# HuiGuanLab/Lite-MKD

Measured on AMD Instinct MI355X. Metric: episodes/sec (5-way 5-shot, 8x224^2 frames), higher is better.
Workload: dtype f32

## Files before the change

### include/lmkd.h

```cpp
#ifndef LMKD_H
#define LMKD_H
#ifdef __cplusplus
extern "C" {
#endif

int lmkd_abi_version(void);
const char* lmkd_last_error(void);
int lmkd_device_check(int device);
int lmkd_set_activation_dtype(int mode);
int lmkd_get_activation_dtype(void);

int lmkd_gemm_f32(char layA, char layB, int M, int N, int K, float alpha, const float* A, long lda, long sA,
                  const float* B, long ldb, long sB, float beta, float* C, long ldc, long sC, const float* bias,
                  int relu, int batch, void* stream);
int lmkd_gemm_set_mode(int mode);
int lmkd_gemm_set_tile(int t);
long lmkd_gemm_ticket_words(void);
int lmkd_gemm_f32_splitk(char layA, char layB, int M, int N, int K, float alpha, const float* A, long lda, long sA,
                         const float* B, long ldb, long sB, float beta, float* C, long ldc, long sC, const float* bias,
                         int relu, int batch, void* workspace, long ws_bytes, unsigned* tickets, void* stream);

long lmkd_conv2d_packed_weight_elems(int Cout, int Cin, int Cs, int KH, int KW, int mode);
int lmkd_conv2d_pack_weights(const float* w_oihw, float* wp, int Cout, int Cin, int Cs, int KH, int KW, int mode ,
                             void* stream);
int lmkd_conv2d_fwd_row_tiles(int N, int H, int W, int Cout, int KH, int KW, int stride, int pad);
int lmkd_conv2d_fwd_row_tiles_cs(int N, int H, int W, int Cs, int Cout, int KH, int KW, int stride, int pad);
int lmkd_set_elementwise_wg_per_cu(int n);
int lmkd_conv_set_compute_dtype(int mode);
typedef struct lmkd_amax_desc {
  const void* x_words;
  const void* dy_words;
  void* out_words;
  const void* ref_words;
  int flags;
} lmkd_amax_desc;
#define LMKD_AMAX_FENCED 1
int lmkd_h2_fence_eval(const void* const* words, void* const* refs, int n, int* flags, void* stream);
long lmkd_conv_h2_fallbacks(void);
int lmkd_amax(const float* x, long n, void* word, void* stream);
long lmkd_amax_words(void);
long lmkd_conv2d_plane_elems(int ncols, int Kp);
long lmkd_conv_h2_launches(void);
int lmkd_conv2d_repack_multi(const float* const* ws, void* const* wfs, const int* dims, int n, void* stream);
int lmkd_conv2d_split_weights(const float* wp, void* wf, int ncols, int Kp, void* stream);
int lmkd_conv_get_compute_dtype(void);
int lmkd_conv_set_wgrad_planes(int on);
int lmkd_conv_set_patch(int on);
int lmkd_conv_set_stem_patch(int on);
int lmkd_conv_set_s2_patch(int on);
int lmkd_conv_set_wgrad_win16(int on);
int lmkd_conv_set_wgrad_stem(int on);
int lmkd_conv_set_wgrad_window(int on);
int lmkd_conv_set_patch16(int on);
int lmkd_conv_set_persistent(int on);
int lmkd_conv_set_xcd_mode(int mode);
int lmkd_conv_set_tile(int id);
int lmkd_conv2d_fwd(const float* x, const float* wp_fwd, float* y, float* stat_partial, int N, int H, int W, int Cs, int Cout,
                    int KH, int KW, int stride, int pad, void* stream);
int lmkd_conv2d_fwd_pre(const float* x_raw, const float* pre_stats, const float* wp_fwd, float* y, float* stat_partial, int N, int H,
                        int W, int Cs, int Cout, int KH, int KW, int stride, int pad, void* stream);
int lmkd_conv2d_fwd_bn(const float* x, const float* wp_fwd, float* y, const float* bn_stats, const float* res , int relu,
                       int N, int H, int W, int Cs, int Cout, int KH, int KW, int stride, int pad, void* stream,
                       const lmkd_amax_desc* amax );
int lmkd_conv2d_bwd_data(const float* dy, const float* wp_dgrad, float* dx, int N, int H, int W, int Cin, int Cout, int KH, int KW,
                         int stride, int pad, int accumulate, void* stream);
int lmkd_conv2d_bwd_data_bn_tiles(int N, int H, int W, int Cin, int Cout, int KH, int KW, int stride, int pad);
int lmkd_conv2d_bwd_data_bn(const float* dy, const float* wp_dgrad, float* dx, const float* bn_x, const float* bn_stats, float* part,
                            int N, int H, int W, int Cin, int Cout, int KH, int KW, int stride, int pad, void* stream);
long lmkd_conv2d_bwd_weight_workspace(int N, int H, int W, int Cs, int Cout, int KH, int KW, int stride, int pad);
int lmkd_conv2d_bwd_weight(const float* x, const float* dy, float* dw_oihw, float* workspace, long ws_bytes, int N, int H, int W,
                           int Cs, int Cin, int Cout, int KH, int KW, int stride, int pad, void* stream);
int lmkd_conv2d_bwd_weight_pre(const float* x_raw, const float* pre_stats, const float* dy, float* dw_oihw, float* workspace,
                               long ws_bytes, int N, int H, int W, int Cs, int Cin, int Cout, int KH, int KW, int stride, int pad,
                               void* stream);

int lmkd_conv2d_plan(int kind, int N, int H, int W, int Cs, int Cin, int Cout, int KH, int KW, int stride, int pad, int* info_host);

int lmkd_conv2d_bwd_weight_acc(const float* x, const float* pre_stats, const float* dy, float* dw_oihw, float* workspace, long ws_bytes,
                               int N, int H, int W, int Cs, int Cin, int Cout, int KH, int KW, int stride, int pad, void* stream);

int lmkd_frames_u8_to_nhwc4(const unsigned char* src, float* dst, const int* crop_y, const int* crop_x, const int* flip, int F, int Hs,
                            int Ws, int H, int W, int frames_per_video, void* stream);
int lmkd_resize_plan(int in_size, int out_size, int* bounds_host, int* coeffs_host);
int lmkd_resize_pass_u8(const unsigned char* src, unsigned char* dst, const int* bounds_dev, const int* coeffs_dev, int ksize, long outer,
                        int n_in, int n_out, long inner, void* stream);
int lmkd_frames_resize_crop_nhwc4(const unsigned char* src, float* dst, const int* bounds_h, const int* coeffs_h, int ksize_h,
                                  const int* bounds_v, const int* coeffs_v, int ksize_v, const int* crop_y, const int* crop_x,
                                  const int* flip, int F, int Hs, int Ws, int Hr, int Wr, int H, int W, int frames_per_video, void* stream);
long lmkd_jpeg_desc_bytes(void);
long lmkd_jpeg_pool_bytes(int n);
const char* lmkd_jpeg_reason(int reason);
int lmkd_jpeg_plan(const unsigned char* data, const long long* offsets, int n, void* descs, void* pool, long pool_cap, long long* info,
                   long long* totals);
int lmkd_jpeg_decode(const unsigned char* data, const void* descs, const void* pool, int n, short* coef, unsigned char* planes,
                     unsigned char* out, int* status, long long max_blocks, long long max_pixels, void* stream);
int lmkd_jpeg_decode_host(const unsigned char* data, const void* descs, const void* pool, int n, short* coef, unsigned char* planes,
                          unsigned char* out, int* status);
int lmkd_nchw3_to_nhwc4(const float* x_nchw, float* y_nhwc4, int N, int H, int W, void* stream, void* amax_words);
long lmkd_ticket_words(void);
int lmkd_bn_finalize(const float* partial, int T, int C, long count, const float* gamma, const float* beta, float* running_mean,
                     float* running_var, float momentum, float eps, float* stats, double* scratch, unsigned* tickets, void* stream,
                     const lmkd_amax_desc* amax );
int lmkd_bn_running_update(float* running_mean, float* running_var, const float* stats, int C, float momentum, void* stream);
int lmkd_bn_running_update_multi(float* const* running_mean, float* const* running_var, const float* const* stats_first,
                                 const float* const* stats_second, const int* C, int n, float momentum, void* stream);
int lmkd_bn_running_update_multi_nbt(float* const* running_mean, float* const* running_var, const float* const* stats_first,
// ... 146 lines not shown
```

### lite-mkd_amd/_lib.py

```python
import ctypes
import os
import re

from . import _audit

_HERE = os.path.dirname(os.path.abspath(__file__))
_ROOT = os.path.dirname(_HERE)
HEADER = os.path.join(_ROOT, "include", "lmkd.h")
LIB_PATH = os.environ.get("LMKD_LIB") or os.path.join(_HERE, "liblmkd_hip.so")

_CT = {
    "int": ctypes.c_int, "long": ctypes.c_long, "float": ctypes.c_float, "char": ctypes.c_char,
    "long long": ctypes.c_longlong, "unsigned long long": ctypes.c_ulonglong,
}


def parse_header(path=HEADER):
    txt = open(path).read()
    txt = re.sub(r"/\*.*?\*/", " ", txt, flags=re.S)
    protos = {}
    for m in re.finditer(r"\b(int|long|const char\s*\*)\s+(lmkd_\w+)\s*\(([^)]*)\)\s*;", txt):
        ret, name, args = m.group(1), m.group(2), m.group(3).strip()
        restype = ctypes.c_char_p if "char" in ret else _CT[ret]
        argtypes = []
        if args and args != "void":
            for a in args.split(","):
                a = a.strip()
                if "*" in a:
                    argtypes.append(ctypes.c_void_p)
                else:
                    toks = a.replace("const ", "").split()
                    ty = " ".join(toks[:-1])
                    argtypes.append(_CT[ty])
        protos[name] = (restype, argtypes)
    return protos


class _Lib:
    def __init__(self):
        if not os.path.exists(LIB_PATH):
            raise RuntimeError(
                "liblmkd_hip.so not found at %s: build it with `python lite-mkd_amd/build.py` "
                "(there is no CPU or PyTorch fallback for the hot path)" % LIB_PATH)
        import torch
        self.cdll = ctypes.CDLL(LIB_PATH)
        self.protos = parse_header()
        for name, (restype, argtypes) in self.protos.items():
            fn = getattr(self.cdll, name)
            fn.restype = restype
            fn.argtypes = argtypes
        if os.environ.get("LMKD_PATCH16"):
            self.cdll.lmkd_conv_set_patch16(int(os.environ["LMKD_PATCH16"]))
        if os.environ.get("LMKD_WGRAD_WINDOW"):
            self.cdll.lmkd_conv_set_wgrad_window(int(os.environ["LMKD_WGRAD_WINDOW"]))
        if os.environ.get("LMKD_CONV_PERSISTENT", "1") == "0":
            self.cdll.lmkd_conv_set_persistent(0)

    def last_error(self):
        return self.cdll.lmkd_last_error().decode()

    def call(self, name, *args):
        if _audit.ON:
            _audit.check(name)
        rc = getattr(self.cdll, name)(*args)
        if rc != 0:
            raise RuntimeError("%s failed (%d): %s" % (name, rc, self.last_error()))

    def value(self, name, *args):
        return getattr(self.cdll, name)(*args)


_lib = None


def lib():
    global _lib
    if _lib is None:
        _lib = _Lib()
    return _lib
```

### lite-mkd_amd/csrc/conv.hip

```cpp
#include "gemm_core.h"
#include <atomic>
#include <mutex>

struct ConvGemmArgs {
  const float* src;
  const float* wpk;
  float* out;
  float* stat_partial;
  int N, Hs, Ws, Cs;
  int Hr, Wr, rows_per_class, tiles_per_class;
  int sh;
  int Ho, Wo, Co, omul;
  int Kp, cps, nclass;
  int n_rt, n_ct, xcd_mode;
  int taps_pm1;
  int grid_step;
  int grid_total;
  int same;
  int halo;
  int accum;
  const float* ep_stats;
  const float* ep_res;
  int ep_relu;
  const float* pre_stats;
// ... 1326 lines not shown
                                    int KH, int KW, int stride, int pad, int accumulate, void* stream) {
  LMKD_REQUIRE(dy && wd && dx, "lmkd_conv2d_bwd_data: null pointer");
  LMKD_REQUIRE(aligned16(dy) && aligned16(wd), "lmkd_conv2d_bwd_data: operands must be 16-byte aligned");
  ConvGemmArgs a;
  if (const int rc = bwd_data_args(a, dy, wd, dx, N, H, W, Cin, Cout, KH, KW, stride, pad, accumulate)) return rc;
  return launch_conv(a, plan_dgrad(a), (hipStream_t)stream);
}

extern "C" int lmkd_conv2d_bwd_data_bn_tiles_seg(int N, int H, int W, int Cin, int Cout, int KH, int KW, int stride, int pad, int seg_n0, int* tiles0) {
  if (stride != 1 || Cout % 32 != 0 || KH * KW > LMKD_MAX_TAPS) return 0;
  ConvGemmArgs a;
  if (bwd_data_args(a, nullptr, nullptr, nullptr, N, H, W, Cin, Cout, KH, KW, stride, pad, 0, seg_n0)) return 0;
  const ConvPlan p = plan_dgrad(a);
  if (!p.bnb_form) return 0;
  if (tiles0) *tiles0 = p.seg_t0;
  return p.tiles_per_class;
}
extern "C" int lmkd_conv2d_bwd_data_bn_tiles(int N, int H, int W, int Cin, int Cout, int KH, int KW, int stride, int pad) {
  return lmkd_conv2d_bwd_data_bn_tiles_seg(N, H, W, Cin, Cout, KH, KW, stride, pad, 0, nullptr);
}
extern "C" int lmkd_conv2d_bwd_data_seg(const float* dy, const float* wd, float* dx, const float* bn_x, const float* bn_stats, float* part, int N,
                                        int H, int W, int Cin, int Cout, int KH, int KW, int stride, int pad, int accumulate, int seg_n0, void* stream,
                                        const lmkd_amax_desc* amax) {
  LMKD_REQUIRE(dy && wd && dx, "lmkd_conv2d_bwd_data_seg: null pointer");
  LMKD_REQUIRE(aligned16(dy) && aligned16(wd), "lmkd_conv2d_bwd_data_seg: operands must be 16-byte aligned");
  LMKD_REQUIRE((bn_x != nullptr) == (bn_stats != nullptr) && (bn_x != nullptr) == (part != nullptr), "lmkd_conv2d_bwd_data_seg: bn_x, bn_stats and part go together");
  ConvGemmArgs a;
  if (const int rc = bwd_data_args(a, dy, wd, dx, N, H, W, Cin, Cout, KH, KW, stride, pad, accumulate, seg_n0, amax)) return rc;
  note_fenced(amax);
  if (bn_x) {
    LMKD_REQUIRE(!accumulate && aligned16(bn_x) && aligned16(bn_stats), "lmkd_conv2d_bwd_data_seg: the fused BatchNorm sums need a plain (non-accumulating) launch and aligned operands");
    a.bnb_x = bn_x; a.bnb_stats = bn_stats; a.stat_partial = part;
  }
  const ConvPlan p = plan_dgrad(a);
  LMKD_REQUIRE(!bn_x || p.bnb_form, "lmkd_conv2d_bwd_data_seg: this launch has no fused form (lmkd_conv2d_bwd_data_bn_tiles_seg returned 0)");
  return launch_conv(a, p, (hipStream_t)stream);
}
extern "C" int lmkd_conv2d_bwd_data_bn(const float* dy, const float* wd, float* dx, const float* bn_x, const float* bn_stats, float* part,
                                       int N, int H, int W, int Cin, int Cout, int KH, int KW, int stride, int pad, void* stream) {
  LMKD_REQUIRE(dy && wd && dx && bn_x && bn_stats && part, "lmkd_conv2d_bwd_data_bn: null pointer");
  LMKD_REQUIRE(aligned16(dy) && aligned16(wd) && aligned16(bn_x) && aligned16(bn_stats), "lmkd_conv2d_bwd_data_bn: operands must be 16-byte aligned");
  ConvGemmArgs a;
  if (const int rc = bwd_data_args(a, dy, wd, dx, N, H, W, Cin, Cout, KH, KW, stride, pad, 0)) return rc;
  a.bnb_x = bn_x; a.bnb_stats = bn_stats; a.stat_partial = part;
  const ConvPlan p = plan_dgrad(a);
  LMKD_REQUIRE(p.bnb_form, "lmkd_conv2d_bwd_data_bn: this launch has no fused form (lmkd_conv2d_bwd_data_bn_tiles returned 0)");
  return launch_conv(a, p, (hipStream_t)stream);
}

static int g_wgrad_planes = 1;
extern "C" int lmkd_conv_set_wgrad_planes(int on) { g_wgrad_planes = on ? 1 : 0; return LMKD_OK; }
static int g_wgrad_win16 = 1;
extern "C" int lmkd_conv_set_wgrad_win16(int on) { g_wgrad_win16 = on ? 1 : 0; return LMKD_OK; }
static int g_wgrad_window = 1;
extern "C" int lmkd_conv_set_wgrad_window(int on) { g_wgrad_window = on < 0 ? 0 : on; return LMKD_OK; }
static inline bool wgrad_win_eligible(int W, int Cs, int Cout, int KH, int KW, int stride, int pad) {
  return g_wgrad_window && g_wgrad_planes && conv_planes() && KH == 3 && KW == 3 && stride == 1 && pad == 1 &&
         Cs % 32 == 0 && 32 + 2 * (W + 1) <= 256;
}
static void wgrad_win_plan(int Mpix, int W, int Cs, int Cout, int* cob, int* splits, int* steps_per_split) {
  *cob = Cout >= 128 ? 4 : 2;
  const int tiles = cdiv(Cout, 32 * *cob) * (Cs / 32);
  const int steps = cdiv(Mpix, LMKD_BK);
  const int warm = cdiv(2 * (W + 1), LMKD_BK);
  const int resident = 256 * ((conv_nprod() >= 6 && *cob == 2) ? 2 : 8 / *cob);
  int sp = g_wgrad_window > 1 ? cdiv(g_wgrad_window, tiles)
                              : std::max((int)(((long)resident * steps + 19600L * 4 / *cob) / (39200L * 4 / *cob)), cdiv(128, tiles));
  const int cap = std::max(1, steps / (12 * warm));
  if (sp > cap) sp = cap;
  *steps_per_split = cdiv(steps, sp);
  *splits = cdiv(steps, *steps_per_split);
}

static void wgrad_plan(int Mpix, int Cout, int Kp, int* splits, int* steps_per_split, int* bm, int* bn, bool planes = false) {
  *bm = Cout <= 64 ? 64 : 128;
  *bn = (Kp % 128 == 0 && Kp >= 1024) ? 128 : 64;
  int per_cu = (*bm == 128 && *bn == 128) ? 2 : ((*bm == 64 && *bn == 64) ? 4 : 3);
  if (planes) {
    if (*bm == 64 && *bn == 128) *bn = 64;
    const int npl = conv_nprod() == 1 ? 1 : 3;
    const long lds = 1L * npl * LMKD_BK * ((*bm * 2 + 64) + (*bn * 2 + 64));
    per_cu = (int)(160 * 1024 / lds);
    if (per_cu > 4) per_cu = 4;
    if (per_cu < 1) per_cu = 1;
  }
  const int tiles = cdiv(Cout, *bm) * cdiv(Kp, *bn);
  const int steps = cdiv(Mpix, LMKD_BK);
  const int slots = 256 * per_cu;
  int best_sp = 1;
  double best_cost = 1e30;
  for (int r = 1; r <= 3; ++r) {
    int sp = (slots * r) / tiles;
    if (sp > steps / 4) sp = steps / 4;
    if (sp < 1) sp = 1;
    const int sps = cdiv(steps, sp);
    sp = cdiv(steps, sps);
    const double rounds = (double)cdiv((long)tiles * sp, slots);
    const double cost = rounds * sps + 1.0 * sp / 8.0;
    if (cost < best_cost) { best_cost = cost; best_sp = sp; }
  }
  if (planes && *bm == 64 && *bn == 64 && best_sp < cdiv(steps, 64)) best_sp = cdiv(steps, 64);
  *steps_per_split = cdiv(steps, best_sp);
  *splits = cdiv(steps, *steps_per_split);
}

static int g_wgrad_stem = 1;
// ... 59 lines not shown
    p.fam = WgFam::Stem;
    p.nprod = conv_nprod(false, maxima);
    p.splits = p.grid = slabs;
  } else if (wgrad_win_eligible(W, Cs, Cout, KH, KW, stride, pad)) {
    const bool w16 = g_wgrad_win16 && conv_nprod(act16) >= 6;
    p.fam = w16 ? WgFam::Win16 : WgFam::Win;
    p.nprod = w16 ? conv_nprod(false, maxima) : conv_nprod(act16);
    wgrad_win_plan(Mpix, W, Cs, Cout, &p.cob, &p.splits, &p.sps0);
    p.splits0 = p.splits;
    if (seg_n0) {
      int sp1, cob1;
      wgrad_win_plan(p.seg_pix0, W, Cs, Cout, &p.cob, &p.splits0, &p.sps0);
      wgrad_win_plan(Mpix - p.seg_pix0, W, Cs, Cout, &cob1, &sp1, &p.sps1);
      p.splits = p.splits0 + sp1;
    }
    p.grid = 8 * cdiv(p.splits, 8) * cdiv(Cout, 32 * p.cob) * (Cs / 32);
  } else {
    const bool planes = conv_planes() && g_wgrad_planes;
    p.fam = planes ? WgFam::Planes : WgFam::Tile;
    p.nprod = planes ? conv_nprod(act16, maxima && !p.smallc && !pre) : (conv_nprod() == 1 ? 1 : 0);
    wgrad_plan(Mpix, Cout, Kp, &p.splits, &p.sps0, &p.bm, &p.bn, planes);
    p.splits0 = p.splits;
    if (seg_n0) {
      int sp1, bm1, bn1;
      wgrad_plan(p.seg_pix0, Cout, Kp, &p.splits0, &p.sps0, &p.bm, &p.bn, planes);
      wgrad_plan(Mpix - p.seg_pix0, Cout, Kp, &sp1, &p.sps1, &bm1, &bn1, planes);
      p.splits = p.splits0 + sp1;
    }
    p.xcd = (g_xcd_mode != 0 && g_xcd_mode != 1 && p.splits >= 32) ? 1 : 0;
    p.grid = (p.xcd ? 8 * cdiv(p.splits, 8) : p.splits) * cdiv(Cout, p.bm) * cdiv(Kp, p.bn);
  }
  p.need = (long)p.splits * Cout * Kp * sizeof(float);
  return p;
}

template <int NPROD, int D, int RLC>
static void launch_stem_wgrad(const StemWgradArgs& w, dim3 grid, size_t lds, hipStream_t s) {
  lds_attr_once<stem_wgrad_kernel<NPROD, D, RLC>>(160 * 1024);
  hipLaunchKernelGGL((stem_wgrad_kernel<NPROD, D, RLC>), grid, dim3(512), lds, s, w);
}
template <int NPROD>
static void launch_stem_wgrad(const StemWgradArgs& w, dim3 grid, size_t lds, hipStream_t s) {
  const bool deep = cdiv(2 * w.Wo, 32) >= 6;
  if (deep && w.RL == 1856) launch_stem_wgrad<NPROD, 6, 1856>(w, grid, lds, s);
  else if (deep) launch_stem_wgrad<NPROD, 6, 0>(w, grid, lds, s);
  else launch_stem_wgrad<NPROD, 2, 0>(w, grid, lds, s);
}
template <int COB>
static void launch_wgrad_win(const WgradWinArgs& w, const WgradPlan& p, bool big, hipStream_t s) {
  const dim3 grid(p.grid);
  if (p.fam == WgFam::Win16) {
    constexpr int JW = COB == 2 ? 1 : 2;
    constexpr int NT = 64 * COB * (2 / JW);
    with_nprod<3, 6, 9>(p.nprod, [&](auto np) {
      if (big && p.pre) hipLaunchKernelGGL((conv_wgrad_win16_kernel<COB, np, 256, true, 9, JW>), grid, dim3(NT), 0, s, w);
      else if (big) hipLaunchKernelGGL((conv_wgrad_win16_kernel<COB, np, 256, false, 9, JW>), grid, dim3(NT), 0, s, w);
      else if (p.pre) hipLaunchKernelGGL((conv_wgrad_win16_kernel<COB, np, 128, true, 9, JW>), grid, dim3(NT), 0, s, w);
      else hipLaunchKernelGGL((conv_wgrad_win16_kernel<COB, np, 128, false, 9, JW>), grid, dim3(NT), 0, s, w);
    });
    return;
  }
  auto go = [&](auto np, auto a16, auto pre) {
    constexpr int NPROD = decltype(np)::value;
    constexpr bool A16 = decltype(a16)::value, PRE = decltype(pre)::value;
    constexpr int TPW = (COB == 2 && NPROD != 1) ? 5 : 9;
    constexpr int NT = 64 * COB * ((9 + TPW - 1) / TPW);
    if (big) hipLaunchKernelGGL((conv_wgrad_win_kernel<COB, NPROD, A16, 256, PRE, TPW>), grid, dim3(NT), 0, s, w);
    else hipLaunchKernelGGL((conv_wgrad_win_kernel<COB, NPROD, A16, 128, PRE, TPW>), grid, dim3(NT), 0, s, w);
  };
  using T = std::true_type;
  using F = std::false_type;
  if (p.act16) go(std::integral_constant<int, 1>{}, T{}, F{});
  else with_nprod<1, 6, 9>(p.nprod, [&](auto np) { if (p.pre) go(np, F{}, T{}); else go(np, F{}, F{}); });
}

template <class CFG>
static void launch_wgrad_planes(const WgradArgs& a, const WgradPlan& p, hipStream_t s) {
  const dim3 grid(p.grid), block(256);
  if (p.act16) {
    if (p.smallc) hipLaunchKernelGGL((conv_wgrad_x3_kernel<CFG, true, 1, false, true>), grid, block, 0, s, a);
    else hipLaunchKernelGGL((conv_wgrad_x3_kernel<CFG, false, 1, false, true>), grid, block, 0, s, a);
  } else if (p.smallc) {
    with_nprod<1, 6, 9>(p.nprod, [&](auto np) { hipLaunchKernelGGL((conv_wgrad_x3_kernel<CFG, true, np, false>), grid, block, 0, s, a); });
  } else if (p.pre) {
    with_nprod<1, 6, 9>(p.nprod, [&](auto np) { hipLaunchKernelGGL((conv_wgrad_x3_kernel<CFG, false, np, true>), grid, block, 0, s, a); });
  } else {
    with_nprod<1, 3, 6, 9>(p.nprod, [&](auto np) { hipLaunchKernelGGL((conv_wgrad_x3_kernel<CFG, false, np, false>), grid, block, 0, s, a); });
  }
}

template <class CFG, bool SM, int THR>
static void launch_wgrad_tile(const WgradArgs& a, const WgradPlan& p, hipStream_t s) {
  const dim3 grid(p.grid);
  if (p.nprod == 1) hipLaunchKernelGGL((conv_wgrad_kernel<CFG, SM, true>), grid, dim3(THR), 0, s, a);
  else if (!SM && p.pre) hipLaunchKernelGGL((conv_wgrad_kernel<CFG, false, false, true>), grid, dim3(THR), 0, s, a);
  else hipLaunchKernelGGL((conv_wgrad_kernel<CFG, SM, false>), grid, dim3(THR), 0, s, a);
}

static int conv2d_bwd_weight_impl(const float* x, const float* pre_stats, const float* dy, float* dw_oihw, float* workspace,
                                  long ws_bytes, int N, int H, int W, int Cs, int Cin, int Cout, int KH, int KW, int stride, int pad,
                                  void* stream, int accumulate = 0, int seg_n0 = 0, const lmkd_amax_desc* am = nullptr) {
  const unsigned* amax_x = am ? (const unsigned*)am->x_words : nullptr;
  const unsigned* amax_dy = am ? (const unsigned*)am->dy_words : nullptr;
  note_fenced(am);
  LMKD_REQUIRE(x && dy && dw_oihw && workspace, "lmkd_conv2d_bwd_weight: null pointer");
  if (seg_n0 <= 0 || seg_n0 >= N) seg_n0 = 0;
  LMKD_REQUIRE(aligned16(x) && aligned16(dy) && aligned16(workspace), "lmkd_conv2d_bwd_weight: operands must be 16-byte aligned");
// ... 145 lines not shown
```

### lite-mkd_amd/csrc/wgrad_win.h

```cpp
#pragma once

struct WgradWinArgs {
  const float* dy;
  const float* x;
  float* slab;
  const float* pre_stats;
  int N, H, W, Cs, Co, Kp;
  int Mpix, steps_total, steps_per_split, splits;
  int n_ct, n_it;
  int seg_pix0, seg_splits0, sps1;
  FastDiv div_hw, div_w;
  const unsigned* h2_xw;
  const unsigned* h2_dyw;
};
template <int COB, int NPROD, bool ACT16, int R, bool PRE = false, int TPW = 9>
__global__ __launch_bounds__(64 * COB * ((9 + TPW - 1) / TPW)) void conv_wgrad_win_kernel(WgradWinArgs a) {
  constexpr int NPL = NPROD == 1 ? 1 : 3;
  static_assert(!ACT16 || (NPROD == 1 && !PRE), "bf16 tensors: one plane, no store-side arithmetic");
  constexpr int THREADS = 64 * COB * ((9 + TPW - 1) / TPW), BM = 32 * COB;
  constexpr int LDA = BM * 2 + 64, A_PLANE = LMKD_BK * LDA;
  constexpr int LDX = 64, X_PLANE = (R + 1) * LDX;
  constexpr int ESZ = ACT16 ? 2 : 4, EPL = ACT16 ? 8 : 4;
  constexpr int A_LPR = BM / EPL, A_RPP = THREADS / A_LPR, A_NI = (LMKD_BK + A_RPP - 1) / A_RPP;
  constexpr int X_LPR = 32 / EPL, X_RPP = THREADS / X_LPR, X_NI = (LMKD_BK + X_RPP - 1) / X_RPP;
// ... 120 lines not shown
#pragma unroll
      for (int ti = 0; ti < TPW; ++ti) {
        const int tp = tap0 + ti;
        if (9 % TPW != 0 && ti >= 9 - TPW * (9 / TPW) && tp >= 9) break;
        const u32x4 a4 = *reinterpret_cast<const u32x4*>(&s_adr[t & 1][tp * LMKD_BK + ((lane >> 5) * 4 + ((lane & 15) >> 2)) * 4]);
        f32x16 c = acc[ti];
#pragma unroll
        for (int g = 0; g < 2; ++g) {
          const unsigned ad[2] = {(g ? a4.z : a4.x) + (unsigned)cb, (g ? a4.w : a4.y) + (unsigned)cb};
          bf16x8 fb[NPL];
#pragma unroll
          for (int p = 0; p < NPL; ++p) {
            const s16x4_t lo = __builtin_amdgcn_ds_read_tr16_b64_v4i16((s16x4_t __attribute__((address_space(3)))*)(s_x + p * X_PLANE + ad[0]));
            const s16x4_t hi = __builtin_amdgcn_ds_read_tr16_b64_v4i16((s16x4_t __attribute__((address_space(3)))*)(s_x + p * X_PLANE + ad[1]));
            union { s16x4_t s[2]; bf16x8 b; } u;
            u.s[0] = lo; u.s[1] = hi;
            fb[p] = u.b;
          }
          if constexpr (NPROD == 1) {
            c = __builtin_amdgcn_mfma_f32_32x32x16_bf16(fa[g][0], fb[0], c, 0, 0, 0);
          } else {
            if (NPROD == 9) {
              c = __builtin_amdgcn_mfma_f32_32x32x16_bf16(fa[g][2], fb[2], c, 0, 0, 0);
              c = __builtin_amdgcn_mfma_f32_32x32x16_bf16(fa[g][1], fb[2], c, 0, 0, 0);
              c = __builtin_amdgcn_mfma_f32_32x32x16_bf16(fa[g][2], fb[1], c, 0, 0, 0);
            }
            c = __builtin_amdgcn_mfma_f32_32x32x16_bf16(fa[g][1], fb[1], c, 0, 0, 0);
            c = __builtin_amdgcn_mfma_f32_32x32x16_bf16(fa[g][0], fb[2], c, 0, 0, 0);
            c = __builtin_amdgcn_mfma_f32_32x32x16_bf16(fa[g][2], fb[0], c, 0, 0, 0);
            c = __builtin_amdgcn_mfma_f32_32x32x16_bf16(fa[g][0], fb[1], c, 0, 0, 0);
            c = __builtin_amdgcn_mfma_f32_32x32x16_bf16(fa[g][1], fb[0], c, 0, 0, 0);
            c = __builtin_amdgcn_mfma_f32_32x32x16_bf16(fa[g][0], fb[0], c, 0, 0, 0);
          }
        }
        acc[ti] = c;
      }
      __syncthreads();
    }
  }

  float* C = a.slab + (long)z * a.Co * a.Kp;
#pragma unroll
  for (int ti = 0; ti < TPW; ++ti) {
    if (9 % TPW != 0 && tap0 + ti >= 9) break;
    const int col = (tap0 + ti) * a.Cs + ci0 + (lane & 31);
#pragma unroll
    for (int e = 0; e < 16; ++e) {
      const int row = co0 + cw * 32 + acc_row(e, lane);
      if (row < a.Co) C[(long)row * a.Kp + col] = acc[ti][e];
    }
  }
}

template <int COB, int NPROD, int R, bool PRE = false, int TPW = 9, int JW = 2>
__global__ __launch_bounds__(64 * COB * ((9 + TPW - 1) / TPW) * (2 / JW), JW == 2 ? 2 : 3) void conv_wgrad_win16_kernel(WgradWinArgs a) {
  static_assert(JW == 2 || (JW == 1 && TPW == 9), "the channel-block split exists for nine taps per wave");
  static_assert(NPROD == 6 || NPROD == 9 || NPROD == 3, "three bf16 planes (6 / 9 products) or two fp16 planes (3 products: conv_patch16.h)");
  constexpr int NPL = NPROD == 3 ? 2 : 3;
  constexpr int THREADS = 64 * COB * ((9 + TPW - 1) / TPW) * (2 / JW), BM = 32 * COB;
  constexpr int LDA = BM * 2 + 32, A_PLANE = LMKD_BK * LDA;
  constexpr int LDX = 64, X_PLANE = (R + 1) * LDX;
  constexpr int A_LPR = BM / 4, A_RPP = THREADS / A_LPR, A_NI = (LMKD_BK + A_RPP - 1) / A_RPP;
  constexpr int X_LPR = 8, X_RPP = THREADS / X_LPR, X_NI = (LMKD_BK + X_RPP - 1) / X_RPP;
  static_assert(THREADS % A_LPR == 0 && THREADS % X_LPR == 0 && (LDA / 32) % 2 == 1, "tile layout");
  __shared__ __attribute__((aligned(16))) unsigned char s_dy[NPL * A_PLANE];
  __shared__ __attribute__((aligned(16))) unsigned char s_x[NPL * X_PLANE];
  __shared__ __attribute__((aligned(16))) unsigned s_adr[2][9 * LMKD_BK];
  const int tid = threadIdx.x, lane = tid & 63, wave = tid >> 6;
  const int tiles = a.n_ct * a.n_it;
  const int xj = blockIdx.x >> 3;
  const int z = (blockIdx.x & 7) + 8 * (xj / tiles);
  if (z >= a.splits) return;
  const int tz = xj - (xj / tiles) * tiles;
  const int co0 = (tz % a.n_ct) * BM, ci0 = (tz / a.n_ct) * 32;
  const WinSlab sl = win_slab(z, a.Mpix, a.steps_per_split, a.seg_pix0, a.seg_splits0, a.sps1);
  const int nk = sl.nk, kend = sl.kend;
  const int halo = a.W + 1;

  const __amdgpu_buffer_rsrc_t rs_dy = x3_rsrc(a.dy, (long)a.Mpix * a.Co * 4);
  const __amdgpu_buffer_rsrc_t rs_x = x3_rsrc(a.x, (long)a.Mpix * a.Cs * 4);
  const int a_c = (tid % A_LPR) * 4, a_r = tid / A_LPR;
  const bool a_cin = co0 + a_c < a.Co;
  const int x_c = (tid % X_LPR) * 4, x_r = tid / X_LPR;
  u32x4 ra[A_NI], rx[X_NI];
  unsigned x_ok = 0;
  float h2_sx = 1.f, h2_sdy = 1.f;
  if constexpr (NPROD == 3) {
    h2_sx = h2_scale(amax_read(a.h2_xw, sl.seg));
    h2_sdy = h2_scale(amax_read(a.h2_dyw, sl.seg));
  }
  float4 psc = float4(), psh = float4();
  if (PRE) {
    psc = *reinterpret_cast<const float4*>(a.pre_stats + (long)sl.seg * 5 * a.Cs + 2 * a.Cs + ci0 + x_c);
    psh = *reinterpret_cast<const float4*>(a.pre_stats + (long)sl.seg * 5 * a.Cs + 3 * a.Cs + ci0 + x_c);
  }
  auto load_dy = [&](int k0) {
#pragma unroll
    for (int i = 0; i < A_NI; ++i) {
      const int p = k0 + a_r + A_RPP * i;
      ra[i] = __builtin_amdgcn_raw_buffer_load_b128(rs_dy, (a_cin && a_r + A_RPP * i < LMKD_BK && p < kend) ? (unsigned)((p * a.Co + co0 + a_c) * 4) : X3_OOB, 0, 0);
    }
  };
  auto load_x = [&](int q0) {
#pragma unroll
    for (int i = 0; i < X_NI; ++i) {
      const int q = q0 + x_r + X_RPP * i;
      const bool ok = x_r + X_RPP * i < LMKD_BK && q >= 0 && q < a.Mpix;
      rx[i] = __builtin_amdgcn_raw_buffer_load_b128(rs_x, ok ? (unsigned)((q * a.Cs + ci0 + x_c) * 4) : X3_OOB, 0, 0);
      if (PRE) x_ok = ok ? (x_ok | (1u << i)) : (x_ok & ~(1u << i));
    }
  };
  auto as_f4 = [](const u32x4& r) { return make_float4(__uint_as_float(r.x), __uint_as_float(r.y), __uint_as_float(r.z), __uint_as_float(r.w)); };
  auto store_dy = [&]() {
#pragma unroll
    for (int i = 0; i < A_NI; ++i) {
      if (a_r + A_RPP * i >= LMKD_BK) continue;
      if constexpr (NPROD == 3) {
        uint2 p0, p1;
        h2_split4(as_f4(ra[i]), h2_sdy, p0, p1);
        unsigned char* d = s_dy + (a_r + A_RPP * i) * LDA + a_c * 2;
        *reinterpret_cast<uint2*>(d) = p0;
        *reinterpret_cast<uint2*>(d + A_PLANE) = p1;
      } else {
        tr_store4<NPL, LDA, A_PLANE>(s_dy, a_r + A_RPP * i, a_c, as_f4(ra[i]));
      }
    }
  };
  auto store_x = [&](int q0) {
#pragma unroll
    for (int i = 0; i < X_NI; ++i) {
      if (x_r + X_RPP * i >= LMKD_BK) continue;
      const int slot = (q0 + x_r + X_RPP * i) & (R - 1);
      float4 v = as_f4(rx[i]);
      if (PRE && ((x_ok >> i) & 1u)) {
        v.x = fmaxf(fmaf(v.x, psc.x, psh.x), 0.f); v.y = fmaxf(fmaf(v.y, psc.y, psh.y), 0.f);
        v.z = fmaxf(fmaf(v.z, psc.z, psh.z), 0.f); v.w = fmaxf(fmaf(v.w, psc.w, psh.w), 0.f);
      }
      uint2 p0, p1, p2;
      if constexpr (NPROD == 3) h2_split4(v, h2_sx, p0, p1); else x3_split4(v, p0, p1, p2);
      unsigned char* d = s_x + slot * LDX + ((x_c * 2) ^ (((slot >> 2) & 1) << 5));
      *reinterpret_cast<uint2*>(d) = p0;
      *reinterpret_cast<uint2*>(d + X_PLANE) = p1;
      if constexpr (NPL == 3) *reinterpret_cast<uint2*>(d + 2 * X_PLANE) = p2;
    }
  };
  auto fill_adr = [&](unsigned* tab, int k0) {
    for (int e = tid; e < 9 * LMKD_BK; e += THREADS) {
      const int tp = e >> 5, r = e & 31;
      const int p = k0 + r;
      unsigned adr = (unsigned)(R * LDX);
      if (p < kend) {
        const int n = fdiv(p, a.div_hw);
        const int rem = p - n * a.H * a.W;
        const int h = fdiv(rem, a.div_w), w = rem - h * a.W;
        const int dh = tp / 3 - 1, dw = tp - (tp / 3) * 3 - 1;
        if ((unsigned)(h + dh) < (unsigned)a.H && (unsigned)(w + dw) < (unsigned)a.W) {
          const int slot = (p + dh * a.W + dw) & (R - 1);
          adr = (unsigned)(slot * LDX + (((slot >> 2) & 1) << 5));
        }
      }
      tab[tp * LMKD_BK + (r & 15) * 2 + (r >> 4)] = adr;
    }
  };

  const int q4 = lane >> 4, idx = lane & 15;
  const int cw = wave % COB, tap0 = JW == 2 ? (wave / COB) * TPW : 0, j0 = JW == 2 ? 0 : wave / COB;
  const int offA = (4 * q4 + (idx >> 2)) * LDA + (cw * 32 + 4 * (idx & 3)) * 2;
  const unsigned cbx = (unsigned)(8 * (idx & 3));
  f32x4 acc[TPW][2][JW];
#pragma unroll
  for (int t = 0; t < TPW; ++t)
#pragma unroll
    for (int i = 0; i < 2; ++i)
#pragma unroll
      for (int j = 0; j < JW; ++j) acc[t][i][j] = f32x4{0.f, 0.f, 0.f, 0.f};

  if (nk > 0) {
    const int kfirst = sl.kfirst;
    for (int j = tid; j < NPL * LDX / 4; j += THREADS)
      reinterpret_cast<unsigned*>(s_x + (j / (LDX / 4)) * X_PLANE + R * LDX)[j % (LDX / 4)] = 0u;
    for (int q0 = kfirst - halo; q0 < kfirst + halo; q0 += LMKD_BK) {
      load_x(q0);
      store_x(q0);
    }
    fill_adr(s_adr[0], kfirst);
    load_dy(kfirst);
    load_x(kfirst + halo);
    for (int t = 0; t < nk; ++t) {
      const int k0 = kfirst + t * LMKD_BK;
      store_dy();
      store_x(k0 + halo);
      __syncthreads();
      if (t + 1 < nk) {
        load_dy(k0 + LMKD_BK);
        load_x(k0 + LMKD_BK + halo);
        fill_adr(s_adr[(t + 1) & 1], k0 + LMKD_BK);
      }
      bf16x8 fa[2][NPL];
#pragma unroll
      for (int i = 0; i < 2; ++i)
#pragma unroll
        for (int p = 0; p < NPL; ++p) {
          const unsigned char* ap = s_dy + p * A_PLANE + offA + i * 32;
          const s16x4_t lo = __builtin_amdgcn_ds_read_tr16_b64_v4i16((s16x4_t __attribute__((address_space(3)))*)ap);
          const s16x4_t hi = __builtin_amdgcn_ds_read_tr16_b64_v4i16((s16x4_t __attribute__((address_space(3)))*)(ap + 16 * LDA));
          union { s16x4_t s[2]; bf16x8 b; } u;
          u.s[0] = lo; u.s[1] = hi;
          fa[i][p] = u.b;
        }
      if constexpr (NPROD == 3 && JW == 2) {
        static_assert(NPROD != 3 || TPW == 9, "all nine taps per wave");
        auto read_fb = [&](int tp, bf16x8 (&fb)[JW][NPL]) {
          const uint2 a2 = *reinterpret_cast<const uint2*>(&s_adr[t & 1][tp * LMKD_BK + (4 * q4 + (idx >> 2)) * 2]);
#pragma unroll
          for (int j = 0; j < JW; ++j) {
            const unsigned lo_a = (a2.x ^ (unsigned)((j0 + j) << 5)) + cbx, hi_a = (a2.y ^ (unsigned)((j0 + j) << 5)) + cbx;
#pragma unroll
            for (int p = 0; p < NPL; ++p) {
              const s16x4_t lo = __builtin_amdgcn_ds_read_tr16_b64_v4i16((s16x4_t __attribute__((address_space(3)))*)(s_x + p * X_PLANE + lo_a));
              const s16x4_t hi = __builtin_amdgcn_ds_read_tr16_b64_v4i16((s16x4_t __attribute__((address_space(3)))*)(s_x + p * X_PLANE + hi_a));
              union { s16x4_t s[2]; bf16x8 b; } u;
              u.s[0] = lo; u.s[1] = hi;
              fb[j][p] = u.b;
            }
          }
        };
        auto mult = [&](int ti, const bf16x8 (&fb)[JW][NPL]) {
#pragma unroll
          for (int j = 0; j < JW; ++j)
#pragma unroll
            for (int i = 0; i < 2; ++i) {
              f32x4 c = acc[ti][i][j];
              c = __builtin_amdgcn_mfma_f32_16x16x32_f16(__builtin_bit_cast(f16x8, fa[i][1]), __builtin_bit_cast(f16x8, fb[j][0]), c, 0, 0, 0);
              c = __builtin_amdgcn_mfma_f32_16x16x32_f16(__builtin_bit_cast(f16x8, fa[i][0]), __builtin_bit_cast(f16x8, fb[j][1]), c, 0, 0, 0);
              c = __builtin_amdgcn_mfma_f32_16x16x32_f16(__builtin_bit_cast(f16x8, fa[i][0]), __builtin_bit_cast(f16x8, fb[j][0]), c, 0, 0, 0);
              acc[ti][i][j] = c;
            }
        };
        bf16x8 fb0[JW][NPL], fb1[JW][NPL];
        read_fb(tap0, fb0);
#pragma unroll
        for (int ti = 0; ti < TPW; ti += 2) {
          if (ti + 1 < TPW) read_fb(tap0 + ti + 1, fb1);
          mult(ti, fb0);
          if (ti + 1 < TPW) {
#pragma unroll
            for (int q = 0; q < JW * NPL * 2 + 1; ++q) {
              __builtin_amdgcn_sched_group_barrier(0x008, 1, 0);
              __builtin_amdgcn_sched_group_barrier(0x100, 1, 0);
            }
            __builtin_amdgcn_sched_group_barrier(0x008, JW * 6 - (JW * NPL * 2 + 1), 0);
            if (ti + 2 < TPW) read_fb(tap0 + ti + 2, fb0);
            mult(ti + 1, fb1);
            if (ti + 2 < TPW) {
#pragma unroll
              for (int q = 0; q < JW * NPL * 2 + 1; ++q) {
                __builtin_amdgcn_sched_group_barrier(0x008, 1, 0);
                __builtin_amdgcn_sched_group_barrier(0x100, 1, 0);
              }
              __builtin_amdgcn_sched_group_barrier(0x008, JW * 6 - (JW * NPL * 2 + 1), 0);
            }
          }
        }
      } else
#pragma unroll
      for (int ti = 0; ti < TPW; ++ti) {
        const int tp = tap0 + ti;
        if (9 % TPW != 0 && ti >= 9 - TPW * (9 / TPW) && tp >= 9) break;
        const uint2 a2 = *reinterpret_cast<const uint2*>(&s_adr[t & 1][tp * LMKD_BK + (4 * q4 + (idx >> 2)) * 2]);
#pragma unroll
        for (int j = 0; j < JW; ++j) {
          bf16x8 fb[NPL];
          const unsigned lo_a = (a2.x ^ (unsigned)((j0 + j) << 5)) + cbx, hi_a = (a2.y ^ (unsigned)((j0 + j) << 5)) + cbx;
#pragma unroll
          for (int p = 0; p < NPL; ++p) {
            const s16x4_t lo = __builtin_amdgcn_ds_read_tr16_b64_v4i16((s16x4_t __attribute__((address_space(3)))*)(s_x + p * X_PLANE + lo_a));
            const s16x4_t hi = __builtin_amdgcn_ds_read_tr16_b64_v4i16((s16x4_t __attribute__((address_space(3)))*)(s_x + p * X_PLANE + hi_a));
            union { s16x4_t s[2]; bf16x8 b; } u;
            u.s[0] = lo; u.s[1] = hi;
            fb[p] = u.b;
          }
#pragma unroll
          for (int i = 0; i < 2; ++i) {
            f32x4 c = acc[ti][i][j];
            if constexpr (NPROD == 3) {
              c = __builtin_amdgcn_mfma_f32_16x16x32_f16(__builtin_bit_cast(f16x8, fa[i][1]), __builtin_bit_cast(f16x8, fb[0]), c, 0, 0, 0);
              c = __builtin_amdgcn_mfma_f32_16x16x32_f16(__builtin_bit_cast(f16x8, fa[i][0]), __builtin_bit_cast(f16x8, fb[1]), c, 0, 0, 0);
              c = __builtin_amdgcn_mfma_f32_16x16x32_f16(__builtin_bit_cast(f16x8, fa[i][0]), __builtin_bit_cast(f16x8, fb[0]), c, 0, 0, 0);
              acc[ti][i][j] = c;
              continue;
            }
            if (NPROD == 9) {
              c = __builtin_amdgcn_mfma_f32_16x16x32_bf16(fa[i][NPL - 1], fb[NPL - 1], c, 0, 0, 0);
              c = __builtin_amdgcn_mfma_f32_16x16x32_bf16(fa[i][1], fb[NPL - 1], c, 0, 0, 0);
              c = __builtin_amdgcn_mfma_f32_16x16x32_bf16(fa[i][NPL - 1], fb[1], c, 0, 0, 0);
            }
            c = __builtin_amdgcn_mfma_f32_16x16x32_bf16(fa[i][1], fb[1], c, 0, 0, 0);
            c = __builtin_amdgcn_mfma_f32_16x16x32_bf16(fa[i][0], fb[NPL - 1], c, 0, 0, 0);
            c = __builtin_amdgcn_mfma_f32_16x16x32_bf16(fa[i][NPL - 1], fb[0], c, 0, 0, 0);
            c = __builtin_amdgcn_mfma_f32_16x16x32_bf16(fa[i][0], fb[1], c, 0, 0, 0);
            c = __builtin_amdgcn_mfma_f32_16x16x32_bf16(fa[i][1], fb[0], c, 0, 0, 0);
            c = __builtin_amdgcn_mfma_f32_16x16x32_bf16(fa[i][0], fb[0], c, 0, 0, 0);
            acc[ti][i][j] = c;
          }
        }
      }
      __syncthreads();
    }
  }

  float* C = a.slab + (long)z * a.Co * a.Kp;
  const float h2_ix = 1.f / h2_sx, h2_idy = 1.f / h2_sdy;
#pragma unroll
  for (int ti = 0; ti < TPW; ++ti) {
    if (9 % TPW != 0 && tap0 + ti >= 9) break;
#pragma unroll
    for (int i = 0; i < 2; ++i)
#pragma unroll
      for (int j = 0; j < JW; ++j) {
        const int col = (tap0 + ti) * a.Cs + ci0 + 16 * (j0 + j) + idx;
#pragma unroll
        for (int e = 0; e < 4; ++e) {
          const int row = co0 + cw * 32 + 16 * i + 4 * q4 + e;
          if (row < a.Co) C[(long)row * a.Kp + col] = NPROD == 3 ? acc[ti][i][j][e] * h2_ix * h2_idy : acc[ti][i][j][e];
        }
      }
  }
}
```

Measured before the change: 50.77.

## Software-pipeline the fp16 two-plane window wgrad kernel with double-buffered dy tiles

Adds a PIPE variant of the 3-product window weight-gradient kernel. It double-buffers the dy LDS tile and spreads the next step's LDS stores, address-table fill and global loads across the nine per-tap MFMA slots, so each step needs one barrier instead of two. The goal is to hide load and store latency behind matrix work. In exchange it doubles dy shared memory, lowers the occupancy hint to 2 blocks, is limited to 256-thread eligible shapes, and adds optional timestamp instrumentation.

```diff
diff --git a/include/lmkd.h b/include/lmkd.h
--- a/include/lmkd.h
+++ b/include/lmkd.h
@@ -52,6 +52,7 @@
 int lmkd_conv_set_wgrad_stem(int on);
 int lmkd_conv_set_wgrad_window(int on);
 int lmkd_conv_set_patch16(int on);
+int lmkd_conv_set_wgrad_pipeline(int on);
 int lmkd_conv_set_persistent(int on);
 int lmkd_conv_set_xcd_mode(int mode);
 int lmkd_conv_set_tile(int id);
diff --git a/lite-mkd_amd/_lib.py b/lite-mkd_amd/_lib.py
--- a/lite-mkd_amd/_lib.py
+++ b/lite-mkd_amd/_lib.py
@@ -55,6 +55,8 @@
             self.cdll.lmkd_conv_set_wgrad_window(int(os.environ["LMKD_WGRAD_WINDOW"]))
         if os.environ.get("LMKD_CONV_PERSISTENT", "1") == "0":
             self.cdll.lmkd_conv_set_persistent(0)
+        if os.environ.get("LMKD_WGRAD_PIPELINE", "1") == "0":
+            self.cdll.lmkd_conv_set_wgrad_pipeline(0)
 
     def last_error(self):
         return self.cdll.lmkd_last_error().decode()
diff --git a/lite-mkd_amd/csrc/conv.hip b/lite-mkd_amd/csrc/conv.hip
--- a/lite-mkd_amd/csrc/conv.hip
+++ b/lite-mkd_amd/csrc/conv.hip
@@ -1402,6 +1402,8 @@
 extern "C" int lmkd_conv_set_wgrad_planes(int on) { g_wgrad_planes = on ? 1 : 0; return LMKD_OK; }
 static int g_wgrad_win16 = 1;
 extern "C" int lmkd_conv_set_wgrad_win16(int on) { g_wgrad_win16 = on ? 1 : 0; return LMKD_OK; }
+static int g_wgrad_pipeline = 1;
+extern "C" int lmkd_conv_set_wgrad_pipeline(int on) { g_wgrad_pipeline = on ? 1 : 0; return LMKD_OK; }
 static int g_wgrad_window = 1;
 extern "C" int lmkd_conv_set_wgrad_window(int on) { g_wgrad_window = on < 0 ? 0 : on; return LMKD_OK; }
 static inline bool wgrad_win_eligible(int W, int Cs, int Cout, int KH, int KW, int stride, int pad) {
@@ -1567,7 +1569,19 @@
   if (p.fam == WgFam::Win16) {
     constexpr int JW = COB == 2 ? 1 : 2;
     constexpr int NT = 64 * COB * (2 / JW);
+    const bool pipe = p.nprod == 3 && g_wgrad_pipeline && (big ? 256 : 128) > 63 + 2 * (w.W + 1) && !(big && COB == 4);
     with_nprod<3, 6, 9>(p.nprod, [&](auto np) {
+      if constexpr (decltype(np)::value == 3) {
+        if (pipe) {
+          if constexpr (COB == 2) {
+            if (big && p.pre) { hipLaunchKernelGGL((conv_wgrad_win16_kernel<COB, 3, 256, true, 9, JW, true>), grid, dim3(NT), 0, s, w); return; }
+            if (big) { hipLaunchKernelGGL((conv_wgrad_win16_kernel<COB, 3, 256, false, 9, JW, true>), grid, dim3(NT), 0, s, w); return; }
+          }
+          if (p.pre) hipLaunchKernelGGL((conv_wgrad_win16_kernel<COB, 3, 128, true, 9, JW, true>), grid, dim3(NT), 0, s, w);
+          else hipLaunchKernelGGL((conv_wgrad_win16_kernel<COB, 3, 128, false, 9, JW, true>), grid, dim3(NT), 0, s, w);
+          return;
+        }
+      }
       if (big && p.pre) hipLaunchKernelGGL((conv_wgrad_win16_kernel<COB, np, 256, true, 9, JW>), grid, dim3(NT), 0, s, w);
       else if (big) hipLaunchKernelGGL((conv_wgrad_win16_kernel<COB, np, 256, false, 9, JW>), grid, dim3(NT), 0, s, w);
       else if (p.pre) hipLaunchKernelGGL((conv_wgrad_win16_kernel<COB, np, 128, true, 9, JW>), grid, dim3(NT), 0, s, w);
diff --git a/lite-mkd_amd/csrc/wgrad_win.h b/lite-mkd_amd/csrc/wgrad_win.h
--- a/lite-mkd_amd/csrc/wgrad_win.h
+++ b/lite-mkd_amd/csrc/wgrad_win.h
@@ -196,10 +196,21 @@
   }
 }
 
-template <int COB, int NPROD, int R, bool PRE = false, int TPW = 9, int JW = 2>
-__global__ __launch_bounds__(64 * COB * ((9 + TPW - 1) / TPW) * (2 / JW), JW == 2 ? 2 : 3) void conv_wgrad_win16_kernel(WgradWinArgs a) {
+#ifndef LMKD_WGRAD_PIPE_VALU
+#define LMKD_WGRAD_PIPE_VALU 3
+#endif
+#ifdef LMKD_STAMPS
+#define WSTAMP(k) do { __builtin_amdgcn_sched_barrier(0); if (t == 5) STAMP(k); __builtin_amdgcn_sched_barrier(0); } while (0)
+#define WSTAMP_WG(i) do { __builtin_amdgcn_sched_barrier(0); __builtin_amdgcn_s_waitcnt(0); wst[i] = __builtin_amdgcn_s_memtime(); __builtin_amdgcn_sched_barrier(0); } while (0)
+#else
+#define WSTAMP(k) do { } while (0)
+#define WSTAMP_WG(i) do { } while (0)
+#endif
+template <int COB, int NPROD, int R, bool PRE = false, int TPW = 9, int JW = 2, bool PIPE = false>
+__global__ __launch_bounds__(64 * COB * ((9 + TPW - 1) / TPW) * (2 / JW), (JW == 2 || PIPE || (R == 256 && NPROD != 3)) ? 2 : 3) void conv_wgrad_win16_kernel(WgradWinArgs a) {
   static_assert(JW == 2 || (JW == 1 && TPW == 9), "the channel-block split exists for nine taps per wave");
   static_assert(NPROD == 6 || NPROD == 9 || NPROD == 3, "three bf16 planes (6 / 9 products) or two fp16 planes (3 products: conv_patch16.h)");
+  static_assert(!PIPE || (NPROD == 3 && TPW == 9), "the pipelined step exists for the two-plane instances");
   constexpr int NPL = NPROD == 3 ? 2 : 3;
   constexpr int THREADS = 64 * COB * ((9 + TPW - 1) / TPW) * (2 / JW), BM = 32 * COB;
   constexpr int LDA = BM * 2 + 32, A_PLANE = LMKD_BK * LDA;
@@ -207,7 +218,8 @@
   constexpr int A_LPR = BM / 4, A_RPP = THREADS / A_LPR, A_NI = (LMKD_BK + A_RPP - 1) / A_RPP;
   constexpr int X_LPR = 8, X_RPP = THREADS / X_LPR, X_NI = (LMKD_BK + X_RPP - 1) / X_RPP;
   static_assert(THREADS % A_LPR == 0 && THREADS % X_LPR == 0 && (LDA / 32) % 2 == 1, "tile layout");
-  __shared__ __attribute__((aligned(16))) unsigned char s_dy[NPL * A_PLANE];
+  static_assert(!PIPE || (A_RPP * A_NI == LMKD_BK && X_RPP * X_NI == LMKD_BK && A_NI + 4 <= TPW), "PIPE: every loader row is a row of the step (no range checks, no branch); one piece of work per tap");
+  __shared__ __attribute__((aligned(16))) unsigned char s_dy[(PIPE ? 2 : 1) * NPL * A_PLANE];
   __shared__ __attribute__((aligned(16))) unsigned char s_x[NPL * X_PLANE];
   __shared__ __attribute__((aligned(16))) unsigned s_adr[2][9 * LMKD_BK];
   const int tid = threadIdx.x, lane = tid & 63, wave = tid >> 6;
@@ -220,6 +232,10 @@
   const WinSlab sl = win_slab(z, a.Mpix, a.steps_per_split, a.seg_pix0, a.seg_splits0, a.sps1);
   const int nk = sl.nk, kend = sl.kend;
   const int halo = a.W + 1;
+#ifdef LMKD_STAMPS
+  unsigned long long wst[4] = {0, 0, 0, 0};
+#endif
+  WSTAMP_WG(0);
 
   const __amdgpu_buffer_rsrc_t rs_dy = x3_rsrc(a.dy, (long)a.Mpix * a.Co * 4);
   const __amdgpu_buffer_rsrc_t rs_x = x3_rsrc(a.x, (long)a.Mpix * a.Cs * 4);
@@ -242,38 +258,38 @@
 #pragma unroll
     for (int i = 0; i < A_NI; ++i) {
       const int p = k0 + a_r + A_RPP * i;
-      ra[i] = __builtin_amdgcn_raw_buffer_load_b128(rs_dy, (a_cin && a_r + A_RPP * i < LMKD_BK && p < kend) ? (unsigned)((p * a.Co + co0 + a_c) * 4) : X3_OOB, 0, 0);
+      ra[i] = __builtin_amdgcn_raw_buffer_load_b128(rs_dy, (a_cin && (PIPE || a_r + A_RPP * i < LMKD_BK) && p < kend) ? (unsigned)((p * a.Co + co0 + a_c) * 4) : X3_OOB, 0, 0);
     }
   };
   auto load_x = [&](int q0) {
 #pragma unroll
     for (int i = 0; i < X_NI; ++i) {
       const int q = q0 + x_r + X_RPP * i;
-      const bool ok = x_r + X_RPP * i < LMKD_BK && q >= 0 && q < a.Mpix;
+      const bool ok = (PIPE || x_r + X_RPP * i < LMKD_BK) && q >= 0 && q < a.Mpix;
       rx[i] = __builtin_amdgcn_raw_buffer_load_b128(rs_x, ok ? (unsigned)((q * a.Cs + ci0 + x_c) * 4) : X3_OOB, 0, 0);
       if (PRE) x_ok = ok ? (x_ok | (1u << i)) : (x_ok & ~(1u << i));
     }
   };
   auto as_f4 = [](const u32x4& r) { return make_float4(__uint_as_float(r.x), __uint_as_float(r.y), __uint_as_float(r.z), __uint_as_float(r.w)); };
-  auto store_dy = [&]() {
-#pragma unroll
-    for (int i = 0; i < A_NI; ++i) {
-      if (a_r + A_RPP * i >= LMKD_BK) continue;
+  auto store_dy = [&](unsigned char* tile, int i0, int i1) {
+#pragma unroll
+    for (int i = i0; i < i1; ++i) {
+      if (!PIPE && a_r + A_RPP * i >= LMKD_BK) continue;
       if constexpr (NPROD == 3) {
         uint2 p0, p1;
         h2_split4(as_f4(ra[i]), h2_sdy, p0, p1);
-        unsigned char* d = s_dy + (a_r + A_RPP * i) * LDA + a_c * 2;
+        unsigned char* d = tile + (a_r + A_RPP * i) * LDA + a_c * 2;
         *reinterpret_cast<uint2*>(d) = p0;
         *reinterpret_cast<uint2*>(d + A_PLANE) = p1;
       } else {
-        tr_store4<NPL, LDA, A_PLANE>(s_dy, a_r + A_RPP * i, a_c, as_f4(ra[i]));
+        tr_store4<NPL, LDA, A_PLANE>(tile, a_r + A_RPP * i, a_c, as_f4(ra[i]));
       }
     }
   };
   auto store_x = [&](int q0) {
 #pragma unroll
     for (int i = 0; i < X_NI; ++i) {
-      if (x_r + X_RPP * i >= LMKD_BK) continue;
+      if (!PIPE && x_r + X_RPP * i >= LMKD_BK) continue;
       const int slot = (q0 + x_r + X_RPP * i) & (R - 1);
       float4 v = as_f4(rx[i]);
       if (PRE && ((x_ok >> i) & 1u)) {
@@ -307,6 +323,27 @@
     }
   };
 
+  auto fill_adr_flat = [&](unsigned* tab, int k0) {
+    static_assert(!PIPE || THREADS == 256, "eight taps x 32 rows per pass");
+    auto fdiv_flat = [](uint32_t v, const FastDiv& f) {
+      const uint32_t m = __umulhi(v, f.mul);
+      return f.d == 1 ? v : (m + ((v - m) >> 1)) >> ((f.sh - 1) & 31);
+    };
+    const int r = tid & 31, p = k0 + r;
+    const int n = fdiv_flat(p, a.div_hw);
+    const int rem = p - n * a.H * a.W;
+    const int h = fdiv_flat(rem, a.div_w), w = rem - h * a.W;
+    auto entry = [&](int tp) {
+      const int dh = tp / 3 - 1, dw = tp - (tp / 3) * 3 - 1;
+      const int slot = (p + dh * a.W + dw) & (R - 1);
+      const bool ok = p < kend && (unsigned)(h + dh) < (unsigned)a.H && (unsigned)(w + dw) < (unsigned)a.W;
+      return ok ? (unsigned)(slot * LDX + (((slot >> 2) & 1) << 5)) : (unsigned)(R * LDX);
+    };
+    const int at = (r & 15) * 2 + (r >> 4);
+    tab[(tid >> 5) * LMKD_BK + at] = entry(tid >> 5);
+    tab[8 * LMKD_BK + at] = entry(8);
+  };
+
   const int q4 = lane >> 4, idx = lane & 15;
   const int cw = wave % COB, tap0 = JW == 2 ? (wave / COB) * TPW : 0, j0 = JW == 2 ? 0 : wave / COB;
   const int offA = (4 * q4 + (idx >> 2)) * LDA + (cw * 32 + 4 * (idx & 3)) * 2;
@@ -330,16 +367,100 @@
     fill_adr(s_adr[0], kfirst);
     load_dy(kfirst);
     load_x(kfirst + halo);
+    if constexpr (PIPE) {
+      constexpr int NMF = JW * 6, NRD = JW * NPL * 2 + 1;
+      store_dy(s_dy, 0, A_NI);
+      store_x(kfirst + halo);
+      load_dy(kfirst + LMKD_BK);
+      load_x(kfirst + LMKD_BK + halo);
+      __syncthreads();
+      WSTAMP_WG(1);
+      unsigned cur = 0, nxt = NPL * A_PLANE;
+      for (int t = 0; t < nk; ++t) {
+        const int k0 = kfirst + t * LMKD_BK;
+        WSTAMP(0);
+        auto piece = [&](int ti) {
+          if (ti < A_NI) store_dy(s_dy + nxt, ti, ti + 1);
+          else if (ti == A_NI) store_x(k0 + LMKD_BK + halo);
+          else if (ti == A_NI + 1) fill_adr_flat(s_adr[(t + 1) & 1], k0 + LMKD_BK);
+          else if (ti == A_NI + 2) load_dy(k0 + 2 * LMKD_BK);
+          else if (ti == A_NI + 3) load_x(k0 + 2 * LMKD_BK + halo);
+        };
+        const unsigned* tab = s_adr[t & 1];
+        bf16x8 fa[2][NPL];
+#pragma unroll
+        for (int i = 0; i < 2; ++i)
+#pragma unroll
+          for (int p = 0; p < NPL; ++p) {
+            const unsigned char* ap = s_dy + cur + p * A_PLANE + offA + i * 32;
+            const s16x4_t lo = __builtin_amdgcn_ds_read_tr16_b64_v4i16((s16x4_t __attribute__((address_space(3)))*)ap);
+            const s16x4_t hi = __builtin_amdgcn_ds_read_tr16_b64_v4i16((s16x4_t __attribute__((address_space(3)))*)(ap + 16 * LDA));
+            union { s16x4_t s[2]; bf16x8 b; } u;
+            u.s[0] = lo; u.s[1] = hi;
+            fa[i][p] = u.b;
+          }
+        auto read_fb = [&](int tp, bf16x8 (&fb)[JW][NPL]) {
+          const uint2 a2 = *reinterpret_cast<const uint2*>(&tab[tp * LMKD_BK + (4 * q4 + (idx >> 2)) * 2]);
+#pragma unroll
+          for (int j = 0; j < JW; ++j) {
+            const unsigned lo_a = (a2.x ^ (unsigned)((j0 + j) << 5)) + cbx, hi_a = (a2.y ^ (unsigned)((j0 + j) << 5)) + cbx;
+#pragma unroll
+            for (int p = 0; p < NPL; ++p) {
+              const s16x4_t lo = __builtin_amdgcn_ds_read_tr16_b64_v4i16((s16x4_t __attribute__((address_space(3)))*)(s_x + p * X_PLANE + lo_a));
+              const s16x4_t hi = __builtin_amdgcn_ds_read_tr16_b64_v4i16((s16x4_t __attribute__((address_space(3)))*)(s_x + p * X_PLANE + hi_a));
+              union { s16x4_t s[2]; bf16x8 b; } u;
+              u.s[0] = lo; u.s[1] = hi;
+              fb[j][p] = u.b;
+            }
+          }
+        };
+        auto mult = [&](int ti, const bf16x8 (&fb)[JW][NPL]) {
+#pragma unroll
+          for (int j = 0; j < JW; ++j)
+#pragma unroll
+            for (int i = 0; i < 2; ++i) {
+              f32x4 c = acc[ti][i][j];
+              c = __builtin_amdgcn_mfma_f32_16x16x32_f16(__builtin_bit_cast(f16x8, fa[i][1]), __builtin_bit_cast(f16x8, fb[j][0]), c, 0, 0, 0);
+              c = __builtin_amdgcn_mfma_f32_16x16x32_f16(__builtin_bit_cast(f16x8, fa[i][0]), __builtin_bit_cast(f16x8, fb[j][1]), c, 0, 0, 0);
+              c = __builtin_amdgcn_mfma_f32_16x16x32_f16(__builtin_bit_cast(f16x8, fa[i][0]), __builtin_bit_cast(f16x8, fb[j][0]), c, 0, 0, 0);
+              acc[ti][i][j] = c;
+            }
+        };
+        bf16x8 fb[2][JW][NPL];
+        read_fb(tap0, fb[0]);
+#pragma unroll
+        for (int ti = 0; ti < TPW; ++ti) {
+          if (ti + 1 < TPW) read_fb(tap0 + ti + 1, fb[(ti + 1) & 1]);
+          piece(ti);
+          mult(ti, fb[ti & 1]);
+#pragma unroll
+          for (int q = 0; q < NMF; ++q) {
+            __builtin_amdgcn_sched_group_barrier(0x008, 1, 0);
+            if (ti + 1 < TPW && q < NRD) __builtin_amdgcn_sched_group_barrier(0x100, 1, 0);
+            __builtin_amdgcn_sched_group_barrier(0x002, LMKD_WGRAD_PIPE_VALU, 0);
+          }
+        }
+        WSTAMP(5);
+        __syncthreads();
+        WSTAMP(6);
+        const unsigned o = cur; cur = nxt; nxt = o;
+      }
+    } else
     for (int t = 0; t < nk; ++t) {
       const int k0 = kfirst + t * LMKD_BK;
-      store_dy();
+      if (t == 0) WSTAMP_WG(1);
+      WSTAMP(0);
+      store_dy(s_dy, 0, A_NI);
       store_x(k0 + halo);
+      WSTAMP(1);
       __syncthreads();
+      WSTAMP(2);
       if (t + 1 < nk) {
         load_dy(k0 + LMKD_BK);
         load_x(k0 + LMKD_BK + halo);
         fill_adr(s_adr[(t + 1) & 1], k0 + LMKD_BK);
       }
+      WSTAMP(3);
       bf16x8 fa[2][NPL];
 #pragma unroll
       for (int i = 0; i < 2; ++i)
@@ -383,6 +504,7 @@
         };
         bf16x8 fb0[JW][NPL], fb1[JW][NPL];
         read_fb(tap0, fb0);
+        WSTAMP(4);
 #pragma unroll
         for (int ti = 0; ti < TPW; ti += 2) {
           if (ti + 1 < TPW) read_fb(tap0 + ti + 1, fb1);
@@ -449,9 +571,12 @@
           }
         }
       }
+      WSTAMP(5);
       __syncthreads();
+      WSTAMP(6);
     }
   }
+  WSTAMP_WG(2);
 
   float* C = a.slab + (long)z * a.Co * a.Kp;
   const float h2_ix = 1.f / h2_sx, h2_idy = 1.f / h2_sdy;
@@ -470,4 +595,10 @@
         }
       }
   }
+  WSTAMP_WG(3);
+#ifdef LMKD_STAMPS
+  if (threadIdx.x == 0 && (blockIdx.x & 63) == 0 && (blockIdx.x >> 6) < 4096) g_lmkd_stamps[(blockIdx.x >> 6) * 8 + 7] = ((wst[1] - wst[0]) & 0xffffffffull) | ((wst[3] - wst[2]) << 32);
+#endif
 }
+#undef WSTAMP
+#undef WSTAMP_WG
```

New measurement: 50.70 (median of 2 runs). About the same (-0.1%).
